# ruotianluo/ImageCaptioning.pytorch

Measured on NVIDIA H100. Metric: captions/sec at beam=5 seq_len=20, higher is better.
Workload: dtype f32 (fp32-grade: split-fp16 x3 tensor-core passes, fp32 accumulate)

## Files before the change

### imagecaptioning.pytorch_b200/csrc/gemm_tc.cu

```cuda
#include <cstdlib>

#include "common.cuh"
#include "ptx.cuh"

namespace capb200 {

namespace {

constexpr int BM = 128;
constexpr int BK = 64;
constexpr int kConsumers = 2;
constexpr int kThreads = 128 * (1 + kConsumers);

struct TcParams {
    CUtensorMap a_hi[kMaxSeg];
    CUtensorMap a_lo[kMaxSeg];
    CUtensorMap w_hi[kMaxSeg];
    CUtensorMap w_lo[kMaxSeg];
    int kblocks[kMaxSeg];
    int nseg;
    int M, N;
    float* C;
    long ldc;
    __half* C_hi;
    __half* C_lo;
    long ldcs;
    const float* bias;
    const float* row_bias;
    long ld_row_bias;
    int rows_per_group;
    int relu;
    const float* residual;
    long ld_res;
    int tiles_m, tiles_n;
    int lstm, H;
    const float* c_prev;
    long ld_cprev;
    const int* src_row;
    float* c_out;
    long ld_cout;
    const float* gather_bias;
    long ld_gb;
    const int* gather_idx;
    float* h_f;
    __half* h_hi;
    __half* h_lo;
    long ld_h;
    unsigned long long* trace;
};

__device__ __forceinline__ unsigned long long gtimer() {
    unsigned long long t;
    asm volatile("mov.u64 %0, %%globaltimer;" : "=l"(t));
    return t;
}
#define CAPB_TRACE(slot) do { if (TRACE && p.trace != nullptr) p.trace[(long)blockIdx.x * 16 + (slot)] = gtimer(); } while (0)

template <int BN, int PASSES>
struct TcCfg {
    static constexpr int kPlanes = (PASSES == 3) ? 2 : 1;
    static constexpr uint32_t kABytes = BM * BK * 2;
    static constexpr uint32_t kWBytes = BN * BK * 2;
    static constexpr uint32_t kStageBytes = kPlanes * (kABytes + kWBytes);
    static constexpr uint32_t kRingBudget = 227 * 1024 - 1024  - 256 ;
    static constexpr int kStages = kRingBudget / kStageBytes >= 8 ? 8 : kRingBudget / kStageBytes;
    static constexpr uint32_t kSmemBytes = kStages * kStageBytes + 1024  + 256 ;
    static_assert(BN == 64 || BN == 128 || BN == 160, "wgmma wrappers exist for N = 64, 128 and 160");
    static_assert(kWBytes % 1024 == 0, "operand tiles must keep the 1024-byte swizzle-atom alignment");
    static_assert(kStages >= 2, "need at least a double buffer");
    static_assert(kSmemBytes <= 227 * 1024, "shared memory of one H100 block");
};

template <int BN>
__device__ __forceinline__ void wgmma_f16(float* acc, uint64_t da, uint64_t db, int scale_d) {
    if (BN == 160) ptx::wgmma_f16_n160(acc, da, db, scale_d);
    else if (BN == 128) ptx::wgmma_f16_n128(acc, da, db, scale_d);
    else ptx::wgmma_f16_n64(acc, da, db, scale_d);
}

enum EpiKind : int {
    kEpiStore = 0,
    kEpiPlanes = 1,
    kEpiLstm = 2,
};

template <int BN>
__device__ __forceinline__ void epi_adds(const TcParams& p, float* acc, int r0, int c0) {
    const int ncol = p.N - c0;
    const int lim[2] = {r0 < p.M ? ncol : 0, r0 + 8 < p.M ? ncol : 0};
    if (p.bias != nullptr) {
        const float* b = p.bias + c0;
#pragma unroll
        for (int j = 0; j < BN / 8; ++j) {
#pragma unroll
            for (int e = 0; e < 2; ++e) {
                if (8 * j + e < ncol) {
                    const float x = __ldg(b + 8 * j + e);
                    acc[4 * j + e] += x;
                    acc[4 * j + 2 + e] += x;
                }
            }
        }
    }
    const float* tab[3][2];
#pragma unroll
    for (int h = 0; h < 2; ++h) {
        const int row = lim[h] > 0 ? r0 + 8 * h : 0;
        tab[0][h] = p.row_bias != nullptr ? p.row_bias + (long)(row / p.rows_per_group) * p.ld_row_bias + c0 : nullptr;
        tab[1][h] = p.gather_bias != nullptr ? p.gather_bias + (long)(lim[h] > 0 ? p.gather_idx[row] : 0) * p.ld_gb + c0 : nullptr;
        tab[2][h] = p.residual != nullptr ? p.residual + (long)row * p.ld_res + c0 : nullptr;
    }
#pragma unroll 1
    for (int t = 0; t < 3; ++t) {
        const float* const t0 = t == 0 ? tab[0][0] : t == 1 ? tab[1][0] : tab[2][0];
        const float* const t1 = t == 0 ? tab[0][1] : t == 1 ? tab[1][1] : tab[2][1];
        if (t0 == nullptr) continue;
#pragma unroll
        for (int j = 0; j < BN / 8; ++j) {
#pragma unroll
            for (int e = 0; e < 4; ++e) {
                const int k = 8 * j + (e & 1);
                if (k < lim[e >> 1]) acc[4 * j + e] += (e >> 1 ? t1 : t0)[k];
            }
        }
    }
    if (p.relu) {
#pragma unroll
        for (int i = 0; i < BN / 2; ++i) acc[i] = fmaxf(acc[i], 0.0f);
    }
}

template <int BN>
__device__ __forceinline__ void epi_lstm(const TcParams& p, const float* acc, int r0, int c0, int lane) {
    const bool odd = lane & 1;
    const int row = r0 + (odd ? 8 : 0);
    const int u0 = c0 >> 2;
    const bool row_ok = row < p.M;
    int src = row;
    if (p.src_row != nullptr && row_ok) src = p.src_row[row];
    const float* cprev = (src >= 0 && p.c_prev != nullptr) ? p.c_prev + (long)src * p.ld_cprev : nullptr;
    float cp[BN / 8];
#pragma unroll
    for (int j = 0; j < BN / 8; ++j) cp[j] = (row_ok && cprev != nullptr && u0 + 2 * j < p.H) ? cprev[u0 + 2 * j] : 0.0f;
    float* const c_out = p.c_out + (long)row * p.ld_cout;
    float* const h_f = p.h_f + (long)row * p.ld_h;
    __half* const h_hi = p.h_hi + (long)row * p.ld_h;
    __half* const h_lo = p.h_lo + (long)row * p.ld_h;
    const bool planes = p.h_hi != nullptr;
#pragma unroll
    for (int j = 0; j < BN / 8; ++j) {
        const float* v = acc + 4 * j;
        const float s0 = __shfl_xor_sync(0xffffffffu, odd ? v[0] : v[2], 1);
        const float s1 = __shfl_xor_sync(0xffffffffu, odd ? v[1] : v[3], 1);
        const float gi = odd ? s0 : v[0], gf = odd ? s1 : v[1], gg = odd ? v[2] : s0, go = odd ? v[3] : s1;
        const int unit = u0 + 2 * j;
        if (row_ok && unit < p.H) {
            const float cn = fast_sigmoid(gf) * cp[j] + fast_sigmoid(gi) * fast_tanh(gg);
            const float hn = fast_sigmoid(go) * fast_tanh(cn);
            c_out[unit] = cn;
            h_f[unit] = hn;
            if (planes) {
                __half hh, hl;
                split_f32(hn, hh, hl);
                h_hi[unit] = hh;
                h_lo[unit] = hl;
            }
        }
    }
}

template <int BN, bool PLANES>
__device__ __forceinline__ void epi_store(const TcParams& p, const float* acc, int r0, int c0) {
    const int ncol = p.N - c0;
#pragma unroll
    for (int h = 0; h < 2; ++h) {
        const int row = r0 + 8 * h;
        if (row >= p.M) continue;
        if (p.C != nullptr) {
            float* const dst = p.C + (long)row * p.ldc + c0;
            if (ncol >= BN && (reinterpret_cast<uintptr_t>(dst) & 7) == 0) {
#pragma unroll
                for (int j = 0; j < BN / 8; ++j) *reinterpret_cast<float2*>(dst + 8 * j) = make_float2(acc[4 * j + 2 * h], acc[4 * j + 2 * h + 1]);
            } else {
#pragma unroll
                for (int j = 0; j < BN / 8; ++j) {
                    if (8 * j < ncol) dst[8 * j] = acc[4 * j + 2 * h];
                    if (8 * j + 1 < ncol) dst[8 * j + 1] = acc[4 * j + 2 * h + 1];
                }
            }
        }
        if (PLANES) {
            __half* const dh = p.C_hi + (long)row * p.ldcs + c0;
            __half* const dl = p.C_lo + (long)row * p.ldcs + c0;
            if (ncol >= BN && ((reinterpret_cast<uintptr_t>(dh) | reinterpret_cast<uintptr_t>(dl)) & 3) == 0) {
#pragma unroll
                for (int j = 0; j < BN / 8; ++j) {
                    __half h0, l0, h1, l1;
                    split_f32(acc[4 * j + 2 * h], h0, l0);
                    split_f32(acc[4 * j + 2 * h + 1], h1, l1);
                    *reinterpret_cast<__half2*>(dh + 8 * j) = __halves2half2(h0, h1);
                    *reinterpret_cast<__half2*>(dl + 8 * j) = __halves2half2(l0, l1);
                }
            } else {
#pragma unroll
                for (int j = 0; j < BN / 8; ++j) {
#pragma unroll
                    for (int e = 0; e < 2; ++e) {
                        __half hi, lo;
                        split_f32(acc[4 * j + 2 * h + e], hi, lo);
                        if (8 * j + e < ncol) { dh[8 * j + e] = hi; dl[8 * j + e] = lo; }
                    }
                }
            }
        }
    }
}

template <int BN, int EPI>
__device__ __forceinline__ void epilogue_tile(const TcParams& p, float* acc, int m0, int n0, int tid) {
    const int warp = tid >> 5, lane = tid & 31;
    const int r0 = m0 + warp * 16 + (lane >> 2);
    const int c0 = n0 + 2 * (lane & 3);
    epi_adds<BN>(p, acc, r0, c0);
    if (EPI == kEpiLstm) epi_lstm<BN>(p, acc, r0, c0, lane);
    else epi_store<BN, EPI == kEpiPlanes>(p, acc, r0, c0);
}

template <int BN, int PASSES, int EPI, bool TRACE = false>
__global__ void __launch_bounds__(kThreads, 1) gemm_tc_kernel(const __grid_constant__ TcParams p) {
    using Cfg = TcCfg<BN, PASSES>;
    extern __shared__ uint8_t smem_raw[];
    uint8_t* smem = reinterpret_cast<uint8_t*>((reinterpret_cast<uintptr_t>(smem_raw) + 1023) & ~uintptr_t(1023));
    uint64_t* full_bar = reinterpret_cast<uint64_t*>(smem + Cfg::kStages * Cfg::kStageBytes);
    uint64_t* empty_bar = full_bar + Cfg::kStages;

    const int wg = threadIdx.x >> 7;
    const int n_tiles = p.tiles_m * p.tiles_n;

    if (threadIdx.x == 0) {
        for (int s = 0; s < p.nseg; ++s) {
            ptx::prefetch_tmap(&p.a_hi[s]);
            ptx::prefetch_tmap(&p.w_hi[s]);
            if (PASSES == 3) {
                ptx::prefetch_tmap(&p.a_lo[s]);
                ptx::prefetch_tmap(&p.w_lo[s]);
            }
        }
        for (int i = 0; i < Cfg::kStages; ++i) {
            ptx::mbar_init(&full_bar[i], 1);
            ptx::mbar_init(&empty_bar[i], kConsumers);
        }
        ptx::fence_mbar_init();
    }
    __syncthreads();
    if (threadIdx.x == 0) CAPB_TRACE(0);

    if (wg == 0) {
        if (threadIdx.x == 0) {
            int stage = 0;
            uint32_t phase = 0;
            for (int t = blockIdx.x; t < n_tiles; t += gridDim.x) {
                const int m0 = (t % p.tiles_m) * BM;
                const int n0 = (t / p.tiles_m) * BN;
                for (int s = 0; s < p.nseg; ++s) {
                    for (int kb = 0; kb < p.kblocks[s]; ++kb) {
                        ptx::mbar_wait(&empty_bar[stage], phase ^ 1);
                        uint8_t* st = smem + stage * Cfg::kStageBytes;
                        uint8_t* a_hi = st;
                        uint8_t* a_lo = st + Cfg::kABytes;
                        uint8_t* w_hi = st + Cfg::kABytes * Cfg::kPlanes;
                        uint8_t* w_lo = st + Cfg::kABytes * 2 + Cfg::kWBytes;
                        ptx::mbar_arrive_expect_tx(&full_bar[stage], Cfg::kStageBytes);
                        ptx::tma_load_2d(a_hi, &p.a_hi[s], &full_bar[stage], kb * BK, m0);
                        ptx::tma_load_2d(w_hi, &p.w_hi[s], &full_bar[stage], kb * BK, n0);
                        if (PASSES == 3) {
                            ptx::tma_load_2d(a_lo, &p.a_lo[s], &full_bar[stage], kb * BK, m0);
                            ptx::tma_load_2d(w_lo, &p.w_lo[s], &full_bar[stage], kb * BK, n0);
                        }
                        if (++stage == Cfg::kStages) { stage = 0; phase ^= 1; }
                    }
                }
            }
        }
    } else {
        const int cw = wg - 1;
        const int tid = threadIdx.x & 127;
        const uint32_t a_off = cw * 64 * 128;
        int stage = 0;
        uint32_t phase = 0;
        int it = 0;
        for (int t = blockIdx.x; t < n_tiles; t += gridDim.x, ++it) {
            const int m0 = (t % p.tiles_m) * BM;
            const int n0 = (t / p.tiles_m) * BN;
            float acc[BN / 2];
#pragma unroll
            for (int i = 0; i < BN / 2; ++i) acc[i] = 0.0f;
            for (int s = 0; s < p.nseg; ++s) {
                for (int kb = 0; kb < p.kblocks[s]; ++kb) {
                    ptx::mbar_wait(&full_bar[stage], phase);
                    if (TRACE && it == 0 && s == 0 && kb == 0 && tid == 0 && cw == 0) CAPB_TRACE(1);
                    const uint32_t st = ptx::smem_u32(smem + stage * Cfg::kStageBytes);
                    const uint32_t a_hi = st + a_off;
                    const uint32_t a_lo = st + Cfg::kABytes + a_off;
                    const uint32_t w_hi = st + Cfg::kABytes * Cfg::kPlanes;
                    const uint32_t w_lo = st + Cfg::kABytes * 2 + Cfg::kWBytes;
#pragma unroll
                    for (int i = 0; i < BN / 2; ++i) ptx::reg_fence(acc[i]);
                    ptx::wgmma_fence();
#pragma unroll
                    for (int k = 0; k < BK / 16; ++k) {
                        const uint32_t koff = k * 32;
                        if (PASSES == 3) {
                            wgmma_f16<BN>(acc, ptx::make_smem_desc_sw128(a_hi + koff), ptx::make_smem_desc_sw128(w_lo + koff), 1);
                            wgmma_f16<BN>(acc, ptx::make_smem_desc_sw128(a_lo + koff), ptx::make_smem_desc_sw128(w_hi + koff), 1);
                        }
                        wgmma_f16<BN>(acc, ptx::make_smem_desc_sw128(a_hi + koff), ptx::make_smem_desc_sw128(w_hi + koff), 1);
                    }
                    ptx::wgmma_commit();
                    ptx::wgmma_wait<0>();
#pragma unroll
                    for (int i = 0; i < BN / 2; ++i) ptx::reg_fence(acc[i]);
                    if (tid == 0) ptx::mbar_arrive(&empty_bar[stage]);
                    if (++stage == Cfg::kStages) { stage = 0; phase ^= 1; }
                }
            }
            if (TRACE && it < 2 && tid == 0 && cw == 0) CAPB_TRACE(2 + it);
            epilogue_tile<BN, EPI>(p, acc, m0 + cw * 64, n0, tid);
            if (TRACE && it < 2 && tid == 0 && cw == 0) CAPB_TRACE(6 + it);
        }
    }
    __syncthreads();
    if (threadIdx.x == 0) CAPB_TRACE(8);
}

typedef CUresult (*EncodeTiledFn)(CUtensorMap*, CUtensorMapDataType, cuuint32_t, void*, const cuuint64_t*, const cuuint64_t*,
                                  const cuuint32_t*, const cuuint32_t*, CUtensorMapInterleave, CUtensorMapSwizzle,
                                  CUtensorMapL2promotion, CUtensorMapFloatOOBfill);

EncodeTiledFn get_encode_fn() {
    static EncodeTiledFn fn = nullptr;
    if (fn == nullptr) {
        void* sym = nullptr;
        cudaDriverEntryPointQueryResult qres;
        if (cudaGetDriverEntryPoint("cuTensorMapEncodeTiled", &sym, cudaEnableDefault, &qres) != cudaSuccess || sym == nullptr) {
            return nullptr;
        }
        fn = reinterpret_cast<EncodeTiledFn>(sym);
    }
    return fn;
}

bool encode_plane(CUtensorMap* map, const __half* base, long rows, long K, long pitch, int box_rows, std::string* err) {
    EncodeTiledFn fn = get_encode_fn();
    if (fn == nullptr) { *err = "cuTensorMapEncodeTiled entry point not available"; return false; }
    cuuint64_t gdim[2] = {static_cast<cuuint64_t>(K), static_cast<cuuint64_t>(rows)};
    cuuint64_t gstride[1] = {static_cast<cuuint64_t>(pitch) * 2};
    cuuint32_t box[2] = {static_cast<cuuint32_t>(BK), static_cast<cuuint32_t>(box_rows)};
    cuuint32_t estr[2] = {1, 1};
    CUresult r = fn(map, CU_TENSOR_MAP_DATA_TYPE_FLOAT16, 2, const_cast<__half*>(base), gdim, gstride, box, estr,
                    CU_TENSOR_MAP_INTERLEAVE_NONE, CU_TENSOR_MAP_SWIZZLE_128B, CU_TENSOR_MAP_L2_PROMOTION_L2_256B,
                    CU_TENSOR_MAP_FLOAT_OOB_FILL_NONE);
    if (r != CUDA_SUCCESS) { *err = "cuTensorMapEncodeTiled failed with CUresult " + std::to_string((int)r); return false; }
    return true;
}

template <int BN, int PASSES, int EPI, bool TRACE = false>
int launch_cfg(const TcParams& prm, cudaStream_t stream) {
    using Cfg = TcCfg<BN, PASSES>;
    static std::atomic<unsigned long long> attr_set{0};
    if (first_use_on_device(attr_set)) {
        CAPB_CHECK_CUDA(cudaFuncSetAttribute(gemm_tc_kernel<BN, PASSES, EPI, TRACE>, cudaFuncAttributeMaxDynamicSharedMemorySize, Cfg::kSmemBytes));
    }
    TcParams prm2 = prm;
    prm2.tiles_n = cdiv(prm.N, BN);
    prm2.tiles_m = cdiv(prm.M, BM);
    const int n_tiles = prm2.tiles_n * prm2.tiles_m;
    const int sms = sm_count();
    gemm_tc_kernel<BN, PASSES, EPI, TRACE><<<n_tiles < sms ? n_tiles : sms, kThreads, Cfg::kSmemBytes, stream>>>(prm2);
    CAPB_CHECK_CUDA(cudaGetLastError());
    return 0;
}

template <int EPI>
int launch_kind(int bn, int passes, const TcParams& prm, cudaStream_t stream) {
    if (prm.trace != nullptr) {
        if (bn == 160) return launch_cfg<160, 3, EPI, true>(prm, stream);
        return bn == 128 ? launch_cfg<128, 3, EPI, true>(prm, stream) : launch_cfg<64, 3, EPI, true>(prm, stream);
    }
    if (bn == 160) return passes == 3 ? launch_cfg<160, 3, EPI>(prm, stream) : launch_cfg<160, 1, EPI>(prm, stream);
    if (bn == 128) return passes == 3 ? launch_cfg<128, 3, EPI>(prm, stream) : launch_cfg<128, 1, EPI>(prm, stream);
    return passes == 3 ? launch_cfg<64, 3, EPI>(prm, stream) : launch_cfg<64, 1, EPI>(prm, stream);
}

}

struct GemmTcPlan {
    TcParams prm;
    int passes;
    int bn;
};

static void fill_epilogue(TcParams& t, const GemmEpilogue& e) {
    t.C = e.C; t.ldc = e.ldc;
    t.C_hi = e.C_hi; t.C_lo = e.C_lo; t.ldcs = e.ldcs;
    t.bias = e.bias; t.row_bias = e.row_bias; t.ld_row_bias = e.ld_row_bias;
    t.rows_per_group = e.rows_per_group < 1 ? 1 : e.rows_per_group;
    t.relu = e.relu;
    t.residual = e.residual; t.ld_res = e.ld_res;
    t.lstm = e.lstm; t.H = e.H;
    t.c_prev = e.c_prev; t.ld_cprev = e.ld_cprev; t.src_row = e.src_row;
    t.c_out = e.c_out; t.ld_cout = e.ld_cout;
    t.gather_bias = e.gather_bias; t.ld_gb = e.ld_gb; t.gather_idx = e.gather_idx;
    t.h_f = e.h_f; t.h_hi = e.h_hi; t.h_lo = e.h_lo; t.ld_h = e.ld_h;
    t.trace = e.trace;
}

bool gemm_tc_supported(const GemmProblem& p, std::string* why) {
    auto bad = [&](const char* m) { if (why) *why = m; return false; };
    if (p.nseg < 1 || p.nseg > kMaxSeg) return bad("1..3 K-segments");
    for (int s = 0; s < p.nseg; ++s) {
        const GemmSeg& g = p.seg[s];
        if (g.A_hi == nullptr || g.W_hi == nullptr) return bad("split planes missing");
        if ((g.lda_h & 7) || (g.ldw_h & 7)) return bad("plane pitch must be a multiple of 8 elements (16 bytes)");
        if ((reinterpret_cast<uintptr_t>(g.A_hi) & 15) || (reinterpret_cast<uintptr_t>(g.W_hi) & 15)) return bad("plane base must be 16-byte aligned");
        if (g.K < 1) return bad("empty K-segment");
    }
    return true;
}

int gemm_tc_tile_n(int M, int N) {
    const int sms = sm_count();
    const int tiles_m = cdiv(M, BM);
    if (tiles_m * cdiv(N, 128) < sms / 2 && N > 64) return 64;
    const long cost128 = (long)cdiv(tiles_m * cdiv(N, 128), sms) * 128;
    const long cost160 = (long)cdiv(tiles_m * cdiv(N, 160), sms) * 160;
    return cost160 < cost128 ? 160 : 128;
}

GemmTcPlan* gemm_tc_plan_create(const GemmProblem& p, int passes) {
    std::string why;
    if (!gemm_tc_supported(p, &why)) { set_error("gemm_tc: unsupported problem: " + why); return nullptr; }
    if (passes != 1 && passes != 3) { set_error("gemm_tc: passes must be 1 or 3"); return nullptr; }
    GemmTcPlan* plan = new GemmTcPlan();
    memset(&plan->prm, 0, sizeof(TcParams));
    plan->passes = passes;
    plan->bn = gemm_tc_tile_n(p.M, p.N);
    TcParams& t = plan->prm;
    t.nseg = p.nseg;
    t.M = p.M;
    t.N = p.N;
    std::string err;
    for (int s = 0; s < p.nseg; ++s) {
        const GemmSeg& g = p.seg[s];
        t.kblocks[s] = cdiv(g.K, BK);
        bool ok = encode_plane(&t.a_hi[s], g.A_hi, p.M, g.K, g.lda_h, BM, &err) &&
                  encode_plane(&t.w_hi[s], g.W_hi, p.N, g.K, g.ldw_h, plan->bn, &err);
        if (ok && passes == 3) {
            if (g.A_lo == nullptr || g.W_lo == nullptr) { err = "lo planes missing for 3-pass mode"; ok = false; }
            ok = ok && encode_plane(&t.a_lo[s], g.A_lo, p.M, g.K, g.lda_h, BM, &err) &&
                 encode_plane(&t.w_lo[s], g.W_lo, p.N, g.K, g.ldw_h, plan->bn, &err);
        }
        if (!ok) { set_error("gemm_tc: " + err); delete plan; return nullptr; }
    }
    fill_epilogue(t, p.epi);
    return plan;
}

void gemm_tc_plan_destroy(GemmTcPlan* plan) { delete plan; }

int gemm_tc_plan_launch(GemmTcPlan* plan, const GemmEpilogue* epi_override, int M_override, cudaStream_t stream) {
    TcParams prm = plan->prm;
    if (epi_override != nullptr) fill_epilogue(prm, *epi_override);
    if (M_override > 0) {
        if (M_override > prm.M) { set_error("gemm_tc: M override exceeds the planned row count"); return 1; }
        prm.M = M_override;
    }
    if (prm.lstm && (prm.N != 4 * prm.H || prm.c_out == nullptr || prm.h_f == nullptr)) {
        set_error("gemm_tc: fused LSTM epilogue needs N == 4H, c_out and h_f");
        return 1;
    }
    if (prm.M <= 0 || prm.N <= 0) return 0;
    const int kind = prm.lstm ? kEpiLstm : prm.C_hi != nullptr ? kEpiPlanes : kEpiStore;
    if (prm.trace != nullptr && plan->passes != 3) { set_error("gemm_tc: the traced kernel is the 3-pass one"); return 1; }
    if (kind == kEpiLstm) return launch_kind<kEpiLstm>(plan->bn, plan->passes, prm, stream);
    if (kind == kEpiPlanes) return launch_kind<kEpiPlanes>(plan->bn, plan->passes, prm, stream);
    return launch_kind<kEpiStore>(plan->bn, plan->passes, prm, stream);
}

}
```

### imagecaptioning.pytorch_b200/csrc/ptx.cuh

```cuda
#pragma once
#include <cstdint>
#include <cuda.h>
#include <cuda_runtime.h>

namespace capb200 {
namespace ptx {

__device__ __forceinline__ uint32_t smem_u32(const void* p) {
    return static_cast<uint32_t>(__cvta_generic_to_shared(p));
}

__device__ __forceinline__ uint32_t elect_one() {
    uint32_t pred = 0;
    asm volatile(
        "{\n\t"
        ".reg .pred P;\n\t"
        "elect.sync _|P, 0xffffffff;\n\t"
        "selp.b32 %0, 1, 0, P;\n\t"
        "}\n"
        : "=r"(pred));
    return pred;
}

__device__ __forceinline__ void mbar_init(uint64_t* bar, uint32_t count) {
    asm volatile("mbarrier.init.shared::cta.b64 [%0], %1;" ::"r"(smem_u32(bar)), "r"(count) : "memory");
}
__device__ __forceinline__ void fence_mbar_init() {
    asm volatile("fence.mbarrier_init.release.cluster;" ::: "memory");
}
__device__ __forceinline__ void fence_proxy_async_smem() {
    asm volatile("fence.proxy.async.shared::cta;" ::: "memory");
}
__device__ __forceinline__ void mbar_arrive_expect_tx(uint64_t* bar, uint32_t bytes) {
    asm volatile("mbarrier.arrive.expect_tx.shared::cta.b64 _, [%0], %1;" ::"r"(smem_u32(bar)), "r"(bytes) : "memory");
}
__device__ __forceinline__ void mbar_arrive(uint64_t* bar) {
    asm volatile("mbarrier.arrive.shared::cta.b64 _, [%0];" ::"r"(smem_u32(bar)) : "memory");
}
__device__ __forceinline__ bool mbar_try_wait(uint64_t* bar, uint32_t parity) {
    uint32_t ok;
    asm volatile(
        "{\n\t"
        ".reg .pred P;\n\t"
        "mbarrier.try_wait.parity.shared::cta.b64 P, [%1], %2;\n\t"
        "selp.b32 %0, 1, 0, P;\n\t"
        "}\n"
        : "=r"(ok)
        : "r"(smem_u32(bar)), "r"(parity)
        : "memory");
    return ok != 0;
}
__device__ __forceinline__ void mbar_wait(uint64_t* bar, uint32_t parity) {
    uint32_t spins = 0;
    while (!mbar_try_wait(bar, parity)) {
        if (++spins > 200000000u) { __trap(); }
    }
}

__device__ __forceinline__ void prefetch_tmap(const CUtensorMap* m) {
    asm volatile("prefetch.tensormap [%0];" ::"l"(reinterpret_cast<uint64_t>(m)) : "memory");
}
__device__ __forceinline__ void tma_load_2d(void* smem_dst, const CUtensorMap* m, uint64_t* bar, int32_t c_inner, int32_t c_outer) {
    asm volatile(
        "cp.async.bulk.tensor.2d.shared::cluster.global.mbarrier::complete_tx::bytes [%0], [%1, {%3, %4}], [%2];"
        ::"r"(smem_u32(smem_dst)), "l"(reinterpret_cast<uint64_t>(m)), "r"(smem_u32(bar)), "r"(c_inner), "r"(c_outer)
        : "memory");
}

__device__ __forceinline__ void bulk_load_1d(void* smem_dst, const void* gsrc, uint32_t bytes, uint64_t* bar) {
    asm volatile("cp.async.bulk.shared::cluster.global.mbarrier::complete_tx::bytes [%0], [%1], %2, [%3];"
                 ::"r"(smem_u32(smem_dst)), "l"(reinterpret_cast<uint64_t>(gsrc)), "r"(bytes), "r"(smem_u32(bar)) : "memory");
}

__device__ __forceinline__ uint32_t cluster_ctaid_x() { uint32_t v; asm volatile("mov.u32 %0, %%cluster_ctaid.x;" : "=r"(v)); return v; }
__device__ __forceinline__ uint32_t cluster_ctaid_y() { uint32_t v; asm volatile("mov.u32 %0, %%cluster_ctaid.y;" : "=r"(v)); return v; }
__device__ __forceinline__ uint32_t cluster_ctarank() { uint32_t v; asm volatile("mov.u32 %0, %%cluster_ctarank;" : "=r"(v)); return v; }
__device__ __forceinline__ void cluster_sync_all() {
    asm volatile("barrier.cluster.arrive.release.aligned;" ::: "memory");
    asm volatile("barrier.cluster.wait.acquire.aligned;" ::: "memory");
}

__device__ __forceinline__ void wgmma_fence() { asm volatile("wgmma.fence.sync.aligned;" ::: "memory"); }
__device__ __forceinline__ void wgmma_commit() { asm volatile("wgmma.commit_group.sync.aligned;" ::: "memory"); }
template <int N>
__device__ __forceinline__ void wgmma_wait() { asm volatile("wgmma.wait_group.sync.aligned %0;" ::"n"(N) : "memory"); }
__device__ __forceinline__ void reg_fence(float& r) { asm volatile("" : "+f"(r)::"memory"); }

__device__ __forceinline__ uint64_t make_smem_desc_sw128(uint32_t smem_addr) {
    uint64_t d = 0;
    d |= static_cast<uint64_t>((smem_addr & 0x3FFFFu) >> 4);
    d |= static_cast<uint64_t>(1) << 16;
    d |= static_cast<uint64_t>(1024u >> 4) << 32;
    d |= static_cast<uint64_t>(1) << 62;
    return d;
}

__device__ __forceinline__ void wgmma_f16_n32(float* d, uint64_t desc_a, uint64_t desc_b, int scale_d) {
    asm volatile(
        "{\n\t.reg .pred p;\n\tsetp.ne.b32 p, %18, 0;\n\t"
        "wgmma.mma_async.sync.aligned.m64n32k16.f32.f16.f16 "
        "{"
        "%0, %1, %2, %3, %4, %5, %6, %7, %8, %9, %10, %11, %12, %13, %14, %15"
        "}, %16, %17, p, 1, 1, 0, 0;\n\t}\n"
        : "+f"(d[0]), "+f"(d[1]), "+f"(d[2]), "+f"(d[3]), "+f"(d[4]), "+f"(d[5]), "+f"(d[6]), "+f"(d[7]),
          "+f"(d[8]), "+f"(d[9]), "+f"(d[10]), "+f"(d[11]), "+f"(d[12]), "+f"(d[13]), "+f"(d[14]), "+f"(d[15])
        : "l"(desc_a), "l"(desc_b), "r"(scale_d));
}
__device__ __forceinline__ void wgmma_f16_n64(float* d, uint64_t desc_a, uint64_t desc_b, int scale_d) {
    asm volatile(
        "{\n\t.reg .pred p;\n\tsetp.ne.b32 p, %34, 0;\n\t"
        "wgmma.mma_async.sync.aligned.m64n64k16.f32.f16.f16 "
        "{"
        "%0, %1, %2, %3, %4, %5, %6, %7, %8, %9, %10, %11, %12, %13, %14, %15, "
        "%16, %17, %18, %19, %20, %21, %22, %23, %24, %25, %26, %27, %28, %29, %30, %31"
        "}, %32, %33, p, 1, 1, 0, 0;\n\t}\n"
        : "+f"(d[0]), "+f"(d[1]), "+f"(d[2]), "+f"(d[3]), "+f"(d[4]), "+f"(d[5]), "+f"(d[6]), "+f"(d[7]),
          "+f"(d[8]), "+f"(d[9]), "+f"(d[10]), "+f"(d[11]), "+f"(d[12]), "+f"(d[13]), "+f"(d[14]), "+f"(d[15]),
          "+f"(d[16]), "+f"(d[17]), "+f"(d[18]), "+f"(d[19]), "+f"(d[20]), "+f"(d[21]), "+f"(d[22]), "+f"(d[23]),
          "+f"(d[24]), "+f"(d[25]), "+f"(d[26]), "+f"(d[27]), "+f"(d[28]), "+f"(d[29]), "+f"(d[30]), "+f"(d[31])
        : "l"(desc_a), "l"(desc_b), "r"(scale_d));
}
__device__ __forceinline__ void wgmma_f16_n128(float* d, uint64_t desc_a, uint64_t desc_b, int scale_d) {
    asm volatile(
        "{\n\t.reg .pred p;\n\tsetp.ne.b32 p, %66, 0;\n\t"
        "wgmma.mma_async.sync.aligned.m64n128k16.f32.f16.f16 "
        "{"
        "%0, %1, %2, %3, %4, %5, %6, %7, %8, %9, %10, %11, %12, %13, %14, %15, "
        "%16, %17, %18, %19, %20, %21, %22, %23, %24, %25, %26, %27, %28, %29, %30, %31, "
        "%32, %33, %34, %35, %36, %37, %38, %39, %40, %41, %42, %43, %44, %45, %46, %47, "
        "%48, %49, %50, %51, %52, %53, %54, %55, %56, %57, %58, %59, %60, %61, %62, %63"
        "}, %64, %65, p, 1, 1, 0, 0;\n\t}\n"
        : "+f"(d[0]), "+f"(d[1]), "+f"(d[2]), "+f"(d[3]), "+f"(d[4]), "+f"(d[5]), "+f"(d[6]), "+f"(d[7]),
          "+f"(d[8]), "+f"(d[9]), "+f"(d[10]), "+f"(d[11]), "+f"(d[12]), "+f"(d[13]), "+f"(d[14]), "+f"(d[15]),
          "+f"(d[16]), "+f"(d[17]), "+f"(d[18]), "+f"(d[19]), "+f"(d[20]), "+f"(d[21]), "+f"(d[22]), "+f"(d[23]),
          "+f"(d[24]), "+f"(d[25]), "+f"(d[26]), "+f"(d[27]), "+f"(d[28]), "+f"(d[29]), "+f"(d[30]), "+f"(d[31]),
          "+f"(d[32]), "+f"(d[33]), "+f"(d[34]), "+f"(d[35]), "+f"(d[36]), "+f"(d[37]), "+f"(d[38]), "+f"(d[39]),
          "+f"(d[40]), "+f"(d[41]), "+f"(d[42]), "+f"(d[43]), "+f"(d[44]), "+f"(d[45]), "+f"(d[46]), "+f"(d[47]),
          "+f"(d[48]), "+f"(d[49]), "+f"(d[50]), "+f"(d[51]), "+f"(d[52]), "+f"(d[53]), "+f"(d[54]), "+f"(d[55]),
          "+f"(d[56]), "+f"(d[57]), "+f"(d[58]), "+f"(d[59]), "+f"(d[60]), "+f"(d[61]), "+f"(d[62]), "+f"(d[63])
        : "l"(desc_a), "l"(desc_b), "r"(scale_d));
}
__device__ __forceinline__ void wgmma_f16_n160(float* d, uint64_t desc_a, uint64_t desc_b, int scale_d) {
    asm volatile(
        "{\n\t.reg .pred p;\n\tsetp.ne.b32 p, %82, 0;\n\t"
        "wgmma.mma_async.sync.aligned.m64n160k16.f32.f16.f16 "
        "{"
        "%0, %1, %2, %3, %4, %5, %6, %7, %8, %9, %10, %11, %12, %13, %14, %15, "
        "%16, %17, %18, %19, %20, %21, %22, %23, %24, %25, %26, %27, %28, %29, %30, %31, "
        "%32, %33, %34, %35, %36, %37, %38, %39, %40, %41, %42, %43, %44, %45, %46, %47, "
        "%48, %49, %50, %51, %52, %53, %54, %55, %56, %57, %58, %59, %60, %61, %62, %63, "
        "%64, %65, %66, %67, %68, %69, %70, %71, %72, %73, %74, %75, %76, %77, %78, %79"
        "}, %80, %81, p, 1, 1, 0, 0;\n\t}\n"
        : "+f"(d[0]), "+f"(d[1]), "+f"(d[2]), "+f"(d[3]), "+f"(d[4]), "+f"(d[5]), "+f"(d[6]), "+f"(d[7]),
          "+f"(d[8]), "+f"(d[9]), "+f"(d[10]), "+f"(d[11]), "+f"(d[12]), "+f"(d[13]), "+f"(d[14]), "+f"(d[15]),
          "+f"(d[16]), "+f"(d[17]), "+f"(d[18]), "+f"(d[19]), "+f"(d[20]), "+f"(d[21]), "+f"(d[22]), "+f"(d[23]),
          "+f"(d[24]), "+f"(d[25]), "+f"(d[26]), "+f"(d[27]), "+f"(d[28]), "+f"(d[29]), "+f"(d[30]), "+f"(d[31]),
          "+f"(d[32]), "+f"(d[33]), "+f"(d[34]), "+f"(d[35]), "+f"(d[36]), "+f"(d[37]), "+f"(d[38]), "+f"(d[39]),
          "+f"(d[40]), "+f"(d[41]), "+f"(d[42]), "+f"(d[43]), "+f"(d[44]), "+f"(d[45]), "+f"(d[46]), "+f"(d[47]),
          "+f"(d[48]), "+f"(d[49]), "+f"(d[50]), "+f"(d[51]), "+f"(d[52]), "+f"(d[53]), "+f"(d[54]), "+f"(d[55]),
          "+f"(d[56]), "+f"(d[57]), "+f"(d[58]), "+f"(d[59]), "+f"(d[60]), "+f"(d[61]), "+f"(d[62]), "+f"(d[63]),
          "+f"(d[64]), "+f"(d[65]), "+f"(d[66]), "+f"(d[67]), "+f"(d[68]), "+f"(d[69]), "+f"(d[70]), "+f"(d[71]),
          "+f"(d[72]), "+f"(d[73]), "+f"(d[74]), "+f"(d[75]), "+f"(d[76]), "+f"(d[77]), "+f"(d[78]), "+f"(d[79])
        : "l"(desc_a), "l"(desc_b), "r"(scale_d));
}
__device__ __forceinline__ void wgmma_tf32_n32(float* d, uint64_t desc_a, uint64_t desc_b, int scale_d) {
    asm volatile(
        "{\n\t.reg .pred p;\n\tsetp.ne.b32 p, %18, 0;\n\t"
        "wgmma.mma_async.sync.aligned.m64n32k8.f32.tf32.tf32 "
        "{"
        "%0, %1, %2, %3, %4, %5, %6, %7, %8, %9, %10, %11, %12, %13, %14, %15"
        "}, %16, %17, p, 1, 1;\n\t}\n"
        : "+f"(d[0]), "+f"(d[1]), "+f"(d[2]), "+f"(d[3]), "+f"(d[4]), "+f"(d[5]), "+f"(d[6]), "+f"(d[7]),
          "+f"(d[8]), "+f"(d[9]), "+f"(d[10]), "+f"(d[11]), "+f"(d[12]), "+f"(d[13]), "+f"(d[14]), "+f"(d[15])
        : "l"(desc_a), "l"(desc_b), "r"(scale_d));
}
__device__ __forceinline__ void wgmma_tf32_n64(float* d, uint64_t desc_a, uint64_t desc_b, int scale_d) {
    asm volatile(
        "{\n\t.reg .pred p;\n\tsetp.ne.b32 p, %34, 0;\n\t"
        "wgmma.mma_async.sync.aligned.m64n64k8.f32.tf32.tf32 "
        "{"
        "%0, %1, %2, %3, %4, %5, %6, %7, %8, %9, %10, %11, %12, %13, %14, %15, "
        "%16, %17, %18, %19, %20, %21, %22, %23, %24, %25, %26, %27, %28, %29, %30, %31"
        "}, %32, %33, p, 1, 1;\n\t}\n"
        : "+f"(d[0]), "+f"(d[1]), "+f"(d[2]), "+f"(d[3]), "+f"(d[4]), "+f"(d[5]), "+f"(d[6]), "+f"(d[7]),
          "+f"(d[8]), "+f"(d[9]), "+f"(d[10]), "+f"(d[11]), "+f"(d[12]), "+f"(d[13]), "+f"(d[14]), "+f"(d[15]),
          "+f"(d[16]), "+f"(d[17]), "+f"(d[18]), "+f"(d[19]), "+f"(d[20]), "+f"(d[21]), "+f"(d[22]), "+f"(d[23]),
          "+f"(d[24]), "+f"(d[25]), "+f"(d[26]), "+f"(d[27]), "+f"(d[28]), "+f"(d[29]), "+f"(d[30]), "+f"(d[31])
        : "l"(desc_a), "l"(desc_b), "r"(scale_d));
}
__device__ __forceinline__ void wgmma_tf32_n128(float* d, uint64_t desc_a, uint64_t desc_b, int scale_d) {
    asm volatile(
        "{\n\t.reg .pred p;\n\tsetp.ne.b32 p, %66, 0;\n\t"
        "wgmma.mma_async.sync.aligned.m64n128k8.f32.tf32.tf32 "
        "{"
        "%0, %1, %2, %3, %4, %5, %6, %7, %8, %9, %10, %11, %12, %13, %14, %15, "
        "%16, %17, %18, %19, %20, %21, %22, %23, %24, %25, %26, %27, %28, %29, %30, %31, "
        "%32, %33, %34, %35, %36, %37, %38, %39, %40, %41, %42, %43, %44, %45, %46, %47, "
        "%48, %49, %50, %51, %52, %53, %54, %55, %56, %57, %58, %59, %60, %61, %62, %63"
        "}, %64, %65, p, 1, 1;\n\t}\n"
        : "+f"(d[0]), "+f"(d[1]), "+f"(d[2]), "+f"(d[3]), "+f"(d[4]), "+f"(d[5]), "+f"(d[6]), "+f"(d[7]),
          "+f"(d[8]), "+f"(d[9]), "+f"(d[10]), "+f"(d[11]), "+f"(d[12]), "+f"(d[13]), "+f"(d[14]), "+f"(d[15]),
          "+f"(d[16]), "+f"(d[17]), "+f"(d[18]), "+f"(d[19]), "+f"(d[20]), "+f"(d[21]), "+f"(d[22]), "+f"(d[23]),
          "+f"(d[24]), "+f"(d[25]), "+f"(d[26]), "+f"(d[27]), "+f"(d[28]), "+f"(d[29]), "+f"(d[30]), "+f"(d[31]),
          "+f"(d[32]), "+f"(d[33]), "+f"(d[34]), "+f"(d[35]), "+f"(d[36]), "+f"(d[37]), "+f"(d[38]), "+f"(d[39]),
          "+f"(d[40]), "+f"(d[41]), "+f"(d[42]), "+f"(d[43]), "+f"(d[44]), "+f"(d[45]), "+f"(d[46]), "+f"(d[47]),
          "+f"(d[48]), "+f"(d[49]), "+f"(d[50]), "+f"(d[51]), "+f"(d[52]), "+f"(d[53]), "+f"(d[54]), "+f"(d[55]),
          "+f"(d[56]), "+f"(d[57]), "+f"(d[58]), "+f"(d[59]), "+f"(d[60]), "+f"(d[61]), "+f"(d[62]), "+f"(d[63])
        : "l"(desc_a), "l"(desc_b), "r"(scale_d));
}

}
}
```

Baseline: 20640.

## Ping-pong consumer warpgroups over whole tiles and vectorize LSTM epilogue stores

Each consumer warpgroup now computes a full 128-row tile with two accumulators and takes alternate tiles, handing off turns through a new mbarrier. One group's epilogue can then overlap the other group's MMA mainloop. Registers are rebalanced with setmaxnreg so the producer gives up registers to the consumers. The LSTM epilogue shuffles gate values so each lane owns contiguous units, which allows float4 and half4 loads and stores. The risks are register pressure from doubled accumulators, and turn_bar needing extra shared memory that the host allocation may not reserve.

```diff
diff --git a/imagecaptioning.pytorch_b200/csrc/gemm_tc.cu b/imagecaptioning.pytorch_b200/csrc/gemm_tc.cu
--- a/imagecaptioning.pytorch_b200/csrc/gemm_tc.cu
+++ b/imagecaptioning.pytorch_b200/csrc/gemm_tc.cu
@@ -130,43 +130,121 @@
     }
 }
 
-template <int BN>
-__device__ __forceinline__ void epi_lstm(const TcParams& p, const float* acc, int r0, int c0, int lane) {
+template <int BN, bool TRACE>
+__device__ __forceinline__ void epi_lstm(const TcParams& p, float* acc, int r0, int c0, int lane, int slot) {
+    constexpr int kRuns = BN / 32;
     const bool odd = lane & 1;
+    const bool upper = lane & 2;
     const int row = r0 + (odd ? 8 : 0);
-    const int u0 = c0 >> 2;
+    const int u0 = ((c0 - 2 * (lane & 3)) >> 2) + (upper ? 4 : 0);
     const bool row_ok = row < p.M;
+    const bool full = u0 + 8 * (kRuns - 1) + 4 <= p.H;
     int src = row;
     if (p.src_row != nullptr && row_ok) src = p.src_row[row];
-    const float* cprev = (src >= 0 && p.c_prev != nullptr) ? p.c_prev + (long)src * p.ld_cprev : nullptr;
+    const float* cprev = (row_ok && src >= 0 && p.c_prev != nullptr) ? p.c_prev + (long)src * p.ld_cprev + u0 : nullptr;
     float cp[BN / 8];
-#pragma unroll
-    for (int j = 0; j < BN / 8; ++j) cp[j] = (row_ok && cprev != nullptr && u0 + 2 * j < p.H) ? cprev[u0 + 2 * j] : 0.0f;
-    float* const c_out = p.c_out + (long)row * p.ld_cout;
-    float* const h_f = p.h_f + (long)row * p.ld_h;
-    __half* const h_hi = p.h_hi + (long)row * p.ld_h;
-    __half* const h_lo = p.h_lo + (long)row * p.ld_h;
-    const bool planes = p.h_hi != nullptr;
+    if (cprev != nullptr && full && (reinterpret_cast<uintptr_t>(cprev) & 15) == 0) {
+#pragma unroll
+        for (int k = 0; k < kRuns; ++k) {
+            const float4 v = *reinterpret_cast<const float4*>(cprev + 8 * k);
+            cp[4 * k] = v.x; cp[4 * k + 1] = v.y; cp[4 * k + 2] = v.z; cp[4 * k + 3] = v.w;
+        }
+    } else {
+#pragma unroll
+        for (int i = 0; i < BN / 8; ++i) {
+            const int du = 8 * (i / 4) + i % 4;
+            cp[i] = (cprev != nullptr && u0 + du < p.H) ? cprev[du] : 0.0f;
+        }
+    }
+    if (TRACE && slot >= 0) {
+        float s = 0.0f;
+#pragma unroll
+        for (int i = 0; i < BN / 8; ++i) s += cp[i];
+        asm volatile("" ::"f"(s));
+        CAPB_TRACE(slot);
+    }
+    __syncwarp();
 #pragma unroll
     for (int j = 0; j < BN / 8; ++j) {
-        const float* v = acc + 4 * j;
+        float* v = acc + 4 * j;
         const float s0 = __shfl_xor_sync(0xffffffffu, odd ? v[0] : v[2], 1);
         const float s1 = __shfl_xor_sync(0xffffffffu, odd ? v[1] : v[3], 1);
         const float gi = odd ? s0 : v[0], gf = odd ? s1 : v[1], gg = odd ? v[2] : s0, go = odd ? v[3] : s1;
-        const int unit = u0 + 2 * j;
-        if (row_ok && unit < p.H) {
-            const float cn = fast_sigmoid(gf) * cp[j] + fast_sigmoid(gi) * fast_tanh(gg);
-            const float hn = fast_sigmoid(go) * fast_tanh(cn);
-            c_out[unit] = cn;
-            h_f[unit] = hn;
-            if (planes) {
-                __half hh, hl;
-                split_f32(hn, hh, hl);
-                h_hi[unit] = hh;
-                h_lo[unit] = hl;
-            }
-        }
-    }
+        v[0] = gi; v[1] = gf; v[2] = gg; v[3] = go;
+    }
+#pragma unroll
+    for (int k = 0; k < kRuns; ++k) {
+#pragma unroll
+        for (int t = 0; t < 2; ++t) {
+            float* x = acc + 4 * (4 * k + t);
+            float* y = acc + 4 * (4 * k + 2 + t);
+#pragma unroll
+            for (int g = 0; g < 4; ++g) {
+                const float keep = upper ? y[g] : x[g];
+                const float recv = __shfl_xor_sync(0xffffffffu, upper ? x[g] : y[g], 2);
+                x[g] = upper ? recv : keep;
+                y[g] = upper ? keep : recv;
+            }
+        }
+    }
+    float cn[BN / 8], hn[BN / 8];
+#pragma unroll
+    for (int i = 0; i < BN / 8; ++i) {
+        const int k = i / 4, o = i % 4;
+        const float* g = acc + 4 * (4 * k + (o >> 1) + 2 * (o & 1));
+        cn[i] = fast_sigmoid(g[1]) * cp[i] + fast_sigmoid(g[0]) * fast_tanh(g[2]);
+        hn[i] = fast_sigmoid(g[3]) * fast_tanh(cn[i]);
+    }
+    if (TRACE && slot >= 0) {
+        float s = 0.0f;
+#pragma unroll
+        for (int i = 0; i < BN / 8; ++i) s += hn[i];
+        asm volatile("" ::"f"(s));
+        CAPB_TRACE(slot + 1);
+    }
+    if (row_ok) {
+        float* const c_out = p.c_out + (long)row * p.ld_cout + u0;
+        float* const h_f = p.h_f + (long)row * p.ld_h + u0;
+        __half* const h_hi = p.h_hi + (long)row * p.ld_h + u0;
+        __half* const h_lo = p.h_lo + (long)row * p.ld_h + u0;
+        const bool planes = p.h_hi != nullptr;
+        const uintptr_t a16 = reinterpret_cast<uintptr_t>(c_out) | reinterpret_cast<uintptr_t>(h_f);
+        const uintptr_t a8 = planes ? reinterpret_cast<uintptr_t>(h_hi) | reinterpret_cast<uintptr_t>(h_lo) : 0;
+        if (full && (a16 & 15) == 0 && (a8 & 7) == 0) {
+#pragma unroll
+            for (int k = 0; k < kRuns; ++k) {
+                const float* c = cn + 4 * k;
+                const float* h = hn + 4 * k;
+                *reinterpret_cast<float4*>(c_out + 8 * k) = make_float4(c[0], c[1], c[2], c[3]);
+                *reinterpret_cast<float4*>(h_f + 8 * k) = make_float4(h[0], h[1], h[2], h[3]);
+                if (planes) {
+                    __half hh[4], hl[4];
+#pragma unroll
+                    for (int o = 0; o < 4; ++o) split_f32(h[o], hh[o], hl[o]);
+                    const __half2 hi01 = __halves2half2(hh[0], hh[1]), hi23 = __halves2half2(hh[2], hh[3]);
+                    const __half2 lo01 = __halves2half2(hl[0], hl[1]), lo23 = __halves2half2(hl[2], hl[3]);
+                    *reinterpret_cast<uint2*>(h_hi + 8 * k) = make_uint2(*reinterpret_cast<const uint32_t*>(&hi01), *reinterpret_cast<const uint32_t*>(&hi23));
+                    *reinterpret_cast<uint2*>(h_lo + 8 * k) = make_uint2(*reinterpret_cast<const uint32_t*>(&lo01), *reinterpret_cast<const uint32_t*>(&lo23));
+                }
+            }
+        } else {
+#pragma unroll
+            for (int i = 0; i < BN / 8; ++i) {
+                const int du = 8 * (i / 4) + i % 4;
+                if (u0 + du < p.H) {
+                    c_out[du] = cn[i];
+                    h_f[du] = hn[i];
+                    if (planes) {
+                        __half hh, hl;
+                        split_f32(hn[i], hh, hl);
+                        h_hi[du] = hh;
+                        h_lo[du] = hl;
+                    }
+                }
+            }
+        }
+    }
+    if (TRACE && slot >= 0) CAPB_TRACE(slot + 2);
 }
 
 template <int BN, bool PLANES>
@@ -216,13 +294,13 @@
     }
 }
 
-template <int BN, int EPI>
-__device__ __forceinline__ void epilogue_tile(const TcParams& p, float* acc, int m0, int n0, int tid) {
+template <int BN, int EPI, bool TRACE>
+__device__ __forceinline__ void epilogue_tile(const TcParams& p, float* acc, int m0, int n0, int tid, int slot) {
     const int warp = tid >> 5, lane = tid & 31;
     const int r0 = m0 + warp * 16 + (lane >> 2);
     const int c0 = n0 + 2 * (lane & 3);
     epi_adds<BN>(p, acc, r0, c0);
-    if (EPI == kEpiLstm) epi_lstm<BN>(p, acc, r0, c0, lane);
+    if (EPI == kEpiLstm) epi_lstm<BN, TRACE>(p, acc, r0, c0, lane, slot);
     else epi_store<BN, EPI == kEpiPlanes>(p, acc, r0, c0);
 }
 
@@ -233,6 +311,7 @@
     uint8_t* smem = reinterpret_cast<uint8_t*>((reinterpret_cast<uintptr_t>(smem_raw) + 1023) & ~uintptr_t(1023));
     uint64_t* full_bar = reinterpret_cast<uint64_t*>(smem + Cfg::kStages * Cfg::kStageBytes);
     uint64_t* empty_bar = full_bar + Cfg::kStages;
+    uint64_t* turn_bar = empty_bar + Cfg::kStages;
 
     const int wg = threadIdx.x >> 7;
     const int n_tiles = p.tiles_m * p.tiles_n;
@@ -248,14 +327,16 @@
         }
         for (int i = 0; i < Cfg::kStages; ++i) {
             ptx::mbar_init(&full_bar[i], 1);
-            ptx::mbar_init(&empty_bar[i], kConsumers);
-        }
+            ptx::mbar_init(&empty_bar[i], 1);
+        }
+        for (int c = 0; c < kConsumers; ++c) ptx::mbar_init(&turn_bar[c], 1);
         ptx::fence_mbar_init();
     }
     __syncthreads();
     if (threadIdx.x == 0) CAPB_TRACE(0);
 
     if (wg == 0) {
+        ptx::setmaxnreg_dec<40>();
         if (threadIdx.x == 0) {
             int stage = 0;
             uint32_t phase = 0;
@@ -283,50 +364,71 @@
             }
         }
     } else {
+        ptx::setmaxnreg_inc<232>();
         const int cw = wg - 1;
         const int tid = threadIdx.x & 127;
-        const uint32_t a_off = cw * 64 * 128;
-        int stage = 0;
-        uint32_t phase = 0;
-        int it = 0;
-        for (int t = blockIdx.x; t < n_tiles; t += gridDim.x, ++it) {
+        constexpr uint32_t kHalf = 64 * 128;
+        int kb_tile = 0;
+        for (int s = 0; s < p.nseg; ++s) kb_tile += p.kblocks[s];
+        int mine = 0;
+        for (int it = cw, t = blockIdx.x + cw * gridDim.x; t < n_tiles; it += 2, t += 2 * gridDim.x, ++mine) {
             const int m0 = (t % p.tiles_m) * BM;
             const int n0 = (t / p.tiles_m) * BN;
-            float acc[BN / 2];
-#pragma unroll
-            for (int i = 0; i < BN / 2; ++i) acc[i] = 0.0f;
+            if (it > 0) ptx::mbar_wait(&turn_bar[cw], (cw == 1 ? mine : mine - 1) & 1);
+            if (TRACE && it == 1 && tid == 0) CAPB_TRACE(4);
+            const long g0 = (long)it * kb_tile;
+            int stage = (int)(g0 % Cfg::kStages);
+            uint32_t phase = (uint32_t)(g0 / Cfg::kStages) & 1;
+            float acc0[BN / 2], acc1[BN / 2];
+#pragma unroll
+            for (int i = 0; i < BN / 2; ++i) { acc0[i] = 0.0f; acc1[i] = 0.0f; }
             for (int s = 0; s < p.nseg; ++s) {
                 for (int kb = 0; kb < p.kblocks[s]; ++kb) {
                     ptx::mbar_wait(&full_bar[stage], phase);
-                    if (TRACE && it == 0 && s == 0 && kb == 0 && tid == 0 && cw == 0) CAPB_TRACE(1);
+                    if (TRACE && it == 0 && s == 0 && kb == 0 && tid == 0) CAPB_TRACE(1);
                     const uint32_t st = ptx::smem_u32(smem + stage * Cfg::kStageBytes);
-                    const uint32_t a_hi = st + a_off;
-                    const uint32_t a_lo = st + Cfg::kABytes + a_off;
+                    const uint32_t a_hi = st;
+                    const uint32_t a_lo = st + Cfg::kABytes;
                     const uint32_t w_hi = st + Cfg::kABytes * Cfg::kPlanes;
                     const uint32_t w_lo = st + Cfg::kABytes * 2 + Cfg::kWBytes;
 #pragma unroll
-                    for (int i = 0; i < BN / 2; ++i) ptx::reg_fence(acc[i]);
+                    for (int i = 0; i < BN / 2; ++i) { ptx::reg_fence(acc0[i]); ptx::reg_fence(acc1[i]); }
                     ptx::wgmma_fence();
 #pragma unroll
                     for (int k = 0; k < BK / 16; ++k) {
                         const uint32_t koff = k * 32;
+                        const uint64_t dwh = ptx::make_smem_desc_sw128(w_hi + koff);
                         if (PASSES == 3) {
-                            wgmma_f16<BN>(acc, ptx::make_smem_desc_sw128(a_hi + koff), ptx::make_smem_desc_sw128(w_lo + koff), 1);
-                            wgmma_f16<BN>(acc, ptx::make_smem_desc_sw128(a_lo + koff), ptx::make_smem_desc_sw128(w_hi + koff), 1);
+                            const uint64_t dwl = ptx::make_smem_desc_sw128(w_lo + koff);
+                            wgmma_f16<BN>(acc0, ptx::make_smem_desc_sw128(a_hi + koff), dwl, 1);
+                            wgmma_f16<BN>(acc1, ptx::make_smem_desc_sw128(a_hi + kHalf + koff), dwl, 1);
+                            wgmma_f16<BN>(acc0, ptx::make_smem_desc_sw128(a_lo + koff), dwh, 1);
+                            wgmma_f16<BN>(acc1, ptx::make_smem_desc_sw128(a_lo + kHalf + koff), dwh, 1);
+                            wgmma_f16<BN>(acc0, ptx::make_smem_desc_sw128(a_hi + koff), dwh, 1);
+                            wgmma_f16<BN>(acc1, ptx::make_smem_desc_sw128(a_hi + kHalf + koff), dwh, 1);
+                        } else {
+                            wgmma_f16<BN>(acc0, ptx::make_smem_desc_sw128(a_hi + koff), dwh, 1);
+                            wgmma_f16<BN>(acc1, ptx::make_smem_desc_sw128(a_hi + kHalf + koff), dwh, 1);
                         }
-                        wgmma_f16<BN>(acc, ptx::make_smem_desc_sw128(a_hi + koff), ptx::make_smem_desc_sw128(w_hi + koff), 1);
                     }
                     ptx::wgmma_commit();
                     ptx::wgmma_wait<0>();
 #pragma unroll
-                    for (int i = 0; i < BN / 2; ++i) ptx::reg_fence(acc[i]);
+                    for (int i = 0; i < BN / 2; ++i) { ptx::reg_fence(acc0[i]); ptx::reg_fence(acc1[i]); }
                     if (tid == 0) ptx::mbar_arrive(&empty_bar[stage]);
                     if (++stage == Cfg::kStages) { stage = 0; phase ^= 1; }
                 }
             }
-            if (TRACE && it < 2 && tid == 0 && cw == 0) CAPB_TRACE(2 + it);
-            epilogue_tile<BN, EPI>(p, acc, m0 + cw * 64, n0, tid);
-            if (TRACE && it < 2 && tid == 0 && cw == 0) CAPB_TRACE(6 + it);
+            if (tid == 0) ptx::mbar_arrive(&turn_bar[cw ^ 1]);
+            if (TRACE && it < 2 && tid == 0) CAPB_TRACE(2 + it);
+#pragma unroll 1
+            for (int h = 0; h < 2; ++h) {
+                const int slot = (TRACE && it < 2 && h == 0 && tid == 0) ? 9 + 3 * it : -1;
+                epilogue_tile<BN, EPI, TRACE>(p, acc0, m0 + 64 * h, n0, tid, slot);
+#pragma unroll
+                for (int i = 0; i < BN / 2; ++i) acc0[i] = acc1[i];
+            }
+            if (TRACE && it < 2 && tid == 0) CAPB_TRACE(6 + it);
         }
     }
     __syncthreads();
diff --git a/imagecaptioning.pytorch_b200/csrc/ptx.cuh b/imagecaptioning.pytorch_b200/csrc/ptx.cuh
--- a/imagecaptioning.pytorch_b200/csrc/ptx.cuh
+++ b/imagecaptioning.pytorch_b200/csrc/ptx.cuh
@@ -57,6 +57,11 @@
     }
 }
 
+template <int N>
+__device__ __forceinline__ void setmaxnreg_dec() { asm volatile("setmaxnreg.dec.sync.aligned.u32 %0;" ::"n"(N)); }
+template <int N>
+__device__ __forceinline__ void setmaxnreg_inc() { asm volatile("setmaxnreg.inc.sync.aligned.u32 %0;" ::"n"(N)); }
+
 __device__ __forceinline__ void prefetch_tmap(const CUtensorMap* m) {
     asm volatile("prefetch.tensormap [%0];" ::"l"(reinterpret_cast<uint64_t>(m)) : "memory");
 }
```

Result: faster. 22670 (median of 6 runs) (+9.9%).
